# raw-lab/mercat2

Measured on AMD Instinct MI355X. Metric: bases/sec at k=31, 10Mx150bp, higher is better.
Workload: dtype u64

## Files before the change

mercat2_amd/csrc/mk_fparse.hip:

```cpp
#include "mk_common.h"
#include "mk_device.h"
#include "mk_env.h"

typedef unsigned long long u64;

#define FP_THREADS 256
#ifndef FP_SUB
#define FP_SUB 8
#endif
#define FP_WAVE_BYTES (FP_SUB * 1024)
#define FP_WAVES (FP_THREADS / 64)

struct FpEntry {
  unsigned a;
  unsigned b;
};
#define FP_A_SEPS(a) (((a) >> 2) & 0x1FFFu)
#define FP_A_FACTS 15
#define FP_F_CONV 0xFu
#define FP_F_LOW_HEAD (1u << 4)
#define FP_F_LOW_TAIL (1u << 5)
#define FP_F_HI (1u << 6)
static_assert(FP_SUB <= 15 && FP_WAVE_BYTES / 2 <= 0x1FFF, "FpEntry.a: bit fields");

__device__ __forceinline__ uint4 load16(const uint8_t* __restrict__ raw, size_t pos, size_t begin, size_t n) {
  uint4 v;
  if (pos + 16 <= n && pos >= begin) {
    v = *reinterpret_cast<const uint4*>(raw + pos);
  } else {
    unsigned w0 = 0, w1 = 0, w2 = 0, w3 = 0;
#pragma unroll
    for (int j = 0; j < 16; ++j) {
      const unsigned c = (pos + j < n && pos + j >= begin) ? (unsigned)raw[pos + j] : 10u;
      const unsigned sh = 8 * (j & 3);
      if (j < 4) w0 |= c << sh; else if (j < 8) w1 |= c << sh; else if (j < 12) w2 |= c << sh; else w3 |= c << sh;
    }
    v = make_uint4(w0, w1, w2, w3);
  }
  return v;
}

__device__ __forceinline__ void classify16(const uint4 v, unsigned& nl, unsigned& gt, unsigned& st, unsigned& low, unsigned& hi) {
#define FP_NZ7(t) ((((t) & 0x7F7F7F7Fu) + 0x7F7F7F7Fu) | (t))
  unsigned a_nl[2] = {0, 0}, a_gt[2] = {0, 0}, a_st[2] = {0, 0}, a_lo[2] = {0, 0}, a_hi[2] = {0, 0};
#pragma unroll
  for (int d = 0; d < 4; ++d) {
    const unsigned xd = d == 0 ? v.x : (d == 1 ? v.y : (d == 2 ? v.z : v.w));
    const unsigned K = (d & 1) ? 0x80402010u : 0x08040201u;
    const unsigned notnl = FP_NZ7(xd ^ 0x0A0A0A0Au) & FP_NZ7(xd ^ 0x0D0D0D0Du);
    const unsigned ge21 = ((xd & 0x7F7F7F7Fu) + 0x5F5F5F5Fu) | xd;
    a_nl[d >> 1] = __builtin_amdgcn_udot4(~notnl & 0x80808080u, K, a_nl[d >> 1], false);
    a_gt[d >> 1] = __builtin_amdgcn_udot4(~FP_NZ7(xd ^ 0x3E3E3E3Eu) & 0x80808080u, K, a_gt[d >> 1], false);
    a_st[d >> 1] = __builtin_amdgcn_udot4(~FP_NZ7(xd ^ 0x2A2A2A2Au) & 0x80808080u, K, a_st[d >> 1], false);
    a_lo[d >> 1] = __builtin_amdgcn_udot4(~ge21 & notnl & 0x80808080u, K, a_lo[d >> 1], false);
    a_hi[d >> 1] = __builtin_amdgcn_udot4(xd & 0x80808080u, K, a_hi[d >> 1], false);
  }
#undef FP_NZ7
  nl = (a_nl[0] >> 7) | ((a_nl[1] >> 7) << 8);
  gt = (a_gt[0] >> 7) | ((a_gt[1] >> 7) << 8);
  st = (a_st[0] >> 7) | ((a_st[1] >> 7) << 8);
  low = (a_lo[0] >> 7) | ((a_lo[1] >> 7) << 8);
  hi = (a_hi[0] >> 7) | ((a_hi[1] >> 7) << 8);
}

__device__ __forceinline__ unsigned lane_header(unsigned start, unsigned nl, unsigned hin, unsigned& hout) {
  const unsigned p = ~nl & 0xFFFFu;
  const unsigned a = start | p, b = start;
  const unsigned sum = a + b + hin;
  const unsigned ci = sum ^ a ^ b;
  hout = (ci >> 16) & 1u;
  return (ci >> 1) & 0xFFFFu;
}

__device__ __forceinline__ unsigned wave_step(unsigned nl, unsigned gt, unsigned st, unsigned low, unsigned prev_nl,
                                              unsigned cin, unsigned& out, unsigned& sep, unsigned& bad_low,
                                              unsigned& last_nl) {
  const int lane = threadIdx.x & 63;
  const unsigned my_last_nl = (nl >> 15) & 1u;
  const unsigned prev = (unsigned)__builtin_amdgcn_update_dpp((int)prev_nl, (int)my_last_nl, 0x138, 0xf, 0xf, false);
  const unsigned ls = ((nl << 1) | prev) & 0xFFFFu;
  const unsigned start = ls & gt;
  unsigned hout0;
  (void)lane_header(start, nl, 0u, hout0);
  const u64 G = __ballot(hout0 != 0);
  const u64 P = __ballot(nl == 0);
  const u64 A = G | P, B = G;
  const u64 sum = A + B + (u64)cin;
  const u64 CI = sum ^ A ^ B;
  const unsigned hin = (unsigned)(CI >> lane) & 1u;
  unsigned hout;
  const unsigned H = lane_header(start, nl, hin, hout);
  sep = start;
  out = ((~H & ~nl & ~st) | start) & 0xFFFFu;
  bad_low = low & ~H;
  last_nl = mk_wave_last(my_last_nl);
  return mk_wave_last(hout);
}

__global__ __launch_bounds__(FP_THREADS) void mk_fparse_summ(const uint8_t* __restrict__ raw, size_t begin, size_t n, size_t nwaves,
                                                             FpEntry* __restrict__ entries, unsigned* __restrict__ masks,
                                                             MkChunkInfo* __restrict__ info, u64* __restrict__ zero_codes,
                                                             u64* __restrict__ zero_bad, size_t code_words, size_t bad_words) {
  const size_t wave = (size_t)blockIdx.x * FP_WAVES + (threadIdx.x >> 6);
  if (wave >= nwaves) return;
  const int lane = threadIdx.x & 63;
  const size_t base = wave * FP_WAVE_BYTES;
  if (zero_codes) {
    constexpr size_t CW = FP_WAVE_BYTES / 32, BW = FP_WAVE_BYTES / 64;
    const size_t c_end = wave + 1 == nwaves ? code_words : (wave + 1) * CW, b_end = wave + 1 == nwaves ? bad_words : (wave + 1) * BW;
    for (size_t w = wave * CW + (size_t)lane; w < c_end && w < code_words; w += 64) zero_codes[w] = 0ull;
    for (size_t w = wave * BW + (size_t)lane; w < b_end && w < bad_words; w += 64) zero_bad[w] = 0ull;
  }
  unsigned prev_nl = (base <= begin) ? 1u : ((raw[base - 1] == 10 || raw[base - 1] == 13) ? 1u : 0u);
  unsigned s0 = 0, s1 = 1, c0 = 0, c1 = 0, seps = 0, any_nl = 0;
  unsigned conv = 0, low_head = 0, low_tail = 0, hi_or = 0;
  unsigned* __restrict__ wmasks = masks + wave * (FP_SUB * 64) + lane;
#pragma unroll 1
  for (int sub = 0; sub < FP_SUB; ++sub) {
    const size_t pos = base + (size_t)sub * 1024 + (size_t)lane * 16;
    unsigned nl, gt, st, low, hi;
    const uint4 v = load16(raw, pos, begin, n);
    classify16(v, nl, gt, st, low, hi);
    hi_or |= v.x | v.y | v.z | v.w;
    unsigned out, sep, bl, last_nl;
    const unsigned e0 = wave_step(nl, gt, st, low, prev_nl, s0, out, sep, bl, last_nl);
    wmasks[sub * 64] = out | (sep << 16);
    c0 += __popc(out);
    seps += __popc(sep);
    if (s1 != s0) {
      unsigned out1, sep1, bl1, ln1;
      const unsigned e1 = wave_step(nl, gt, st, low, prev_nl, s1, out1, sep1, bl1, ln1);
      c1 += __popc(out1);
      s1 = e1;
      ++conv;
      low_head |= bl;
    } else {
      c1 += __popc(out);
      s1 = e0;
      low_tail |= bl;
    }
    s0 = e0;
    any_nl |= (__ballot(nl != 0) != 0) ? 1u : 0u;
    prev_nl = last_nl;
  }
  c0 = mk_wave_sum(c0);
  c1 = mk_wave_sum(c1);
  seps = mk_wave_sum(seps);
  const unsigned facts = conv | (__ballot(low_head != 0) ? FP_F_LOW_HEAD : 0u) | (__ballot(low_tail != 0) ? FP_F_LOW_TAIL : 0u) |
                         (__ballot((hi_or & 0x80808080u) != 0) ? FP_F_HI : 0u);
  if (lane == 0) {
    entries[wave].a = any_nl | (s0 << 1) | (seps << 2) | (facts << FP_A_FACTS);
    entries[wave].b = c0 | (c1 << 16);
  }
}

struct FpScan {
  u64 off;
  unsigned st;
  unsigned facts;
};

__global__ __launch_bounds__(1024) void mk_fparse_scan(const FpEntry* __restrict__ entries, size_t nwaves,
                                                       FpScan* __restrict__ scan, MkChunkInfo* __restrict__ info,
                                                       u64* __restrict__ bad) {
  const size_t per = (nwaves + 1023) / 1024;
  const size_t lo = (size_t)threadIdx.x * per, hi = (lo + per < nwaves) ? lo + per : nwaves;
  unsigned e0 = 0, e1 = 1, has = 0;
  u64 c0 = 0, c1 = 0, nsep = 0;
  for (size_t w0 = lo; w0 < hi; w0 += 8) {
    FpEntry en[8];
#pragma unroll
    for (int i = 0; i < 8; ++i) en[i] = (w0 + i < hi) ? entries[w0 + i] : FpEntry{0u, 0u};
#pragma unroll
    for (int i = 0; i < 8; ++i) {
      if (w0 + i >= hi) break;
      const unsigned wnl = en[i].a & 1u, wx0 = (en[i].a >> 1) & 1u;
      const unsigned k0 = en[i].b & 0xFFFFu, k1 = en[i].b >> 16;
      nsep += FP_A_SEPS(en[i].a);
      c0 += e0 ? k1 : k0;
      c1 += e1 ? k1 : k0;
      e0 = wnl ? wx0 : (e0 | wx0);
      e1 = wnl ? wx0 : (e1 | wx0);
      has |= wnl;
    }
  }
  __shared__ unsigned long long w_G[16], w_P[16];
  __shared__ unsigned w_cin[16];
  __shared__ u64 w_cnt[16], w_sep[16];
  const int lane = threadIdx.x & 63, wv = threadIdx.x >> 6;
  const u64 G = __ballot(e0 != 0), P = __ballot(has == 0);
  if (lane == 0) { w_G[wv] = G; w_P[wv] = P; }
  __syncthreads();
  if (threadIdx.x == 0) {
    unsigned cin = 0;
    for (int w = 0; w < 16; ++w) {
      w_cin[w] = cin;
      const u64 A = w_G[w] | w_P[w], B = w_G[w];
      const u64 sum = A + B + cin;
      const u64 CI = sum ^ A ^ B;
      cin = (unsigned)((w_G[w] >> 63) | ((w_P[w] >> 63) & (CI >> 63))) & 1u;
    }
  }
  __syncthreads();
  unsigned q;
  {
    const u64 A = G | P, B = G;
    const u64 CI = (A + B + (u64)w_cin[wv]) ^ A ^ B;
    q = (unsigned)(CI >> lane) & 1u;
  }
  const u64 mine = q ? c1 : c0;
  u64 inc = mine;
#pragma unroll
  for (int d = 1; d < 64; d <<= 1) {
    const u64 up = __shfl_up(inc, d);
    if (lane >= d) inc += up;
  }
  for (int d = 32; d > 0; d >>= 1) nsep += __shfl_down(nsep, d);
  if (lane == 63) w_cnt[wv] = inc;
  if (lane == 0) w_sep[wv] = nsep;
  __syncthreads();
  u64 off = inc - mine;
  u64 total = 0, seps = 0;
#pragma unroll
  for (int w = 0; w < 16; ++w) {
    const u64 v = w_cnt[w];
    if (w < wv) off += v;
    total += v;
    seps += w_sep[w];
  }
  if (threadIdx.x == 0) {
    info->seq_len = total;
    info->symbols = total - seps;
    if (bad) {
      if (total & 63) atomicOr(&bad[total >> 6], ~0ull << (total & 63));
      const u64 w = (total + 63) >> 6;
      bad[w] = ~0ull;
      bad[w + 1] = ~0ull;
      bad[w + 2] = ~0ull;
    }
  }
  for (size_t w0 = lo; w0 < hi; w0 += 8) {
    FpEntry en[8];
#pragma unroll
    for (int i = 0; i < 8; ++i) en[i] = (w0 + i < hi) ? entries[w0 + i] : FpEntry{0u, 0u};
#pragma unroll
    for (int i = 0; i < 8; ++i) {
      if (w0 + i >= hi) break;
      scan[w0 + i].off = off;
      scan[w0 + i].st = q;
      scan[w0 + i].facts = en[i].a >> FP_A_FACTS;
      const unsigned wnl = en[i].a & 1u, wx0 = (en[i].a >> 1) & 1u;
      off += q ? (en[i].b >> 16) : (en[i].b & 0xFFFFu);
      q = wnl ? wx0 : (q | wx0);
    }
  }
}

__global__ __launch_bounds__(FP_THREADS) void mk_fparse_emit(const uint8_t* __restrict__ raw, size_t begin, size_t n, size_t nwaves,
                                                             const FpScan* __restrict__ scan, const unsigned* __restrict__ masks,
                                                             uint8_t* __restrict__ seq, MkChunkInfo* __restrict__ info,
                                                             u64* __restrict__ codes, u64* __restrict__ bad, int write_seq,
                                                             int classic) {
  __shared__ __attribute__((aligned(16))) uint8_t stage[FP_WAVES][64 + FP_WAVE_BYTES + 32 + 64 + 256];
  const int wv = threadIdx.x >> 6;
  const size_t wave = (size_t)blockIdx.x * FP_WAVES + wv;
  if (wave >= nwaves) return;
  const int lane = threadIdx.x & 63;
  const size_t base = wave * FP_WAVE_BYTES;
  const FpScan sc = scan[wave];
  const unsigned shift = (unsigned)(sc.off & 15);
  uint8_t* __restrict__ lds = stage[wv] + 64;
  const bool all_classic = classic || (sc.facts & FP_F_HI);
  const int nclassic = __builtin_amdgcn_readfirstlane(all_classic ? FP_SUB : (sc.st ? (int)(sc.facts & FP_F_CONV) : 0));
  unsigned prev_nl = (nclassic == 0 || base <= begin) ? 1u : ((raw[base - 1] == 10 || raw[base - 1] == 13) ? 1u : 0u);
  unsigned state = sc.st;
  unsigned filled = 0;
  int nbad = 0;
  unsigned flag_low = all_classic ? 0u : (sc.facts & (sc.st ? FP_F_LOW_TAIL : (FP_F_LOW_TAIL | FP_F_LOW_HEAD)));
  unsigned nhi = 0;
  const unsigned* __restrict__ wmasks = masks + wave * (FP_SUB * 64) + lane;
  uint4 v_next = load16(raw, base + (size_t)lane * 16, begin, n);
  unsigned m_next = wmasks[0];
#pragma unroll 1
  for (int sub = 0; sub < FP_SUB; ++sub) {
    const uint4 v = v_next;
    const unsigned m = m_next;
    if (sub + 1 < FP_SUB) {
      v_next = load16(raw, base + (size_t)(sub + 1) * 1024 + (size_t)lane * 16, begin, n);
      m_next = wmasks[(sub + 1) * 64];
    }
    unsigned out, sep;
    if (sub < nclassic) {
      unsigned nl, gt, st, low, hi, bl, last_nl;
      classify16(v, nl, gt, st, low, hi);
      state = wave_step(nl, gt, st, low, prev_nl, state, out, sep, bl, last_nl);
      prev_nl = last_nl;
      flag_low |= bl;
      nhi += __popc(hi & out & ~sep);
    } else {
      out = m & 0xFFFFu;
      sep = m >> 16;
    }
    const unsigned cnt = __popc(out);
    nbad -= (int)__popc(sep);
    const unsigned inc = mk_wave_scan_incl(cnt);
    unsigned at = shift + filled + inc - cnt;
#define FP_BYTE(j) ((uint8_t)(((j) < 4 ? v.x : ((j) < 8 ? v.y : ((j) < 12 ? v.z : v.w))) >> (8 * ((j) & 3))))
    if (out == 0xFFFFu && sep == 0) {
#ifdef FP_BYTE_STORES
#pragma unroll
      for (int j = 0; j < 16; ++j) lds[at + j] = FP_BYTE(j);
#else
      __builtin_memcpy(lds + at, &v, 16);
#endif
    } else if (out) {
      const unsigned dump = FP_WAVE_BYTES + 32 + 64 + ((unsigned)lane << 2);
      unsigned a = at;
#pragma unroll
      for (int j = 0; j < 16; ++j) {
        const unsigned kept = (out >> j) & 1u;
        lds[kept ? a : dump] = FP_BYTE(j);
        a += kept;
      }
      for (unsigned sp = sep; sp; sp &= sp - 1) lds[at + __popc(out & ((1u << (__ffs(sp) - 1)) - 1u))] = (uint8_t)MK_SEP;
    }
#undef FP_BYTE
    filled += mk_wave_last(inc);
  }
  __builtin_amdgcn_wave_barrier();
  __threadfence_block();
  uint8_t* __restrict__ dst = seq + (sc.off - shift);
  const unsigned end = shift + filled;
  for (unsigned c = (unsigned)lane * 16; write_seq && c < end; c += 64 * 16) {
    if (c >= shift && c + 16 <= end) {
      *reinterpret_cast<uint4*>(dst + c) = *reinterpret_cast<const uint4*>(lds + c);
    } else {
      const unsigned lo = c < shift ? shift : c;
      const unsigned hi = c + 16 < end ? c + 16 : end;
      for (unsigned j = lo; j < hi; ++j) dst[j] = lds[j];
    }
  }
  if (codes) {
    const u64 g0 = sc.off, g1 = sc.off + filled;
    for (u64 b = (g0 >> 6) + lane; b < ((g1 + 63) >> 6); b += 64) {
      const u64 s_lo = b << 6, s_hi = s_lo + 64;
      const u64 lo = s_lo > g0 ? s_lo : g0, hi = s_hi < g1 ? s_hi : g1;
      u64 w0 = 0, w1 = 0, bd = 0;
      unsigned b8[8] = {0, 0, 0, 0, 0, 0, 0, 0};
      const uint4* p = reinterpret_cast<const uint4*>(lds + (long)shift + (long)(s_lo - g0));
#pragma unroll
      for (int q = 0; q < 4; ++q) {
        const uint4 v = p[q];
#pragma unroll
        for (int d = 0; d < 4; ++d) {
          const unsigned xd = d == 0 ? v.x : (d == 1 ? v.y : (d == 2 ? v.z : v.w));
          const unsigned c = ((xd >> 1) & 0x03030303u) ^ ((xd >> 2) & 0x01010101u);
          const unsigned df = __builtin_amdgcn_perm(0u, 0x54474341u, c) ^ xd;
          const unsigned nz = (((df & 0x7F7F7F7Fu) + 0x7F7F7F7Fu) | df) & 0x80808080u;
          const unsigned m1 = nz >> 7;
          const unsigned ck = c & ~(m1 | (m1 << 1));
          const unsigned g = __builtin_amdgcn_udot4(ck, 0x01041040u, 0u, false);
          const int idx = q * 4 + d;
          if (idx < 8) w0 |= (u64)g << (56 - 8 * idx); else w1 |= (u64)g << (56 - 8 * (idx - 8));
          b8[idx >> 1] = __builtin_amdgcn_udot4(nz, (idx & 1) ? 0x80402010u : 0x08040201u, b8[idx >> 1], false);
        }
      }
#pragma unroll
      for (int i = 0; i < 8; ++i) bd |= (u64)(b8[i] >> 7) << (8 * i);
      if (hi - lo == 64) {
        codes[2 * b] = w0;
        codes[2 * b + 1] = w1;
        bad[b] = bd;
      } else {
        const unsigned a = (unsigned)(lo - s_lo), e = (unsigned)(hi - s_lo);
        const u64 inmask = ((e - a) >= 64 ? ~0ull : ((1ull << (e - a)) - 1)) << a;
        const unsigned a0 = a < 32 ? a : 32, e0 = e < 32 ? e : 32, a1 = a > 32 ? a - 32 : 0, e1 = e > 32 ? e - 32 : 0;
        const u64 m0 = a0 < e0 ? ((~0ull >> (2 * a0)) & ~(e0 == 32 ? 0ull : (~0ull >> (2 * e0)))) : 0ull;
        const u64 m1 = a1 < e1 ? ((~0ull >> (2 * a1)) & ~(e1 == 32 ? 0ull : (~0ull >> (2 * e1)))) : 0ull;
        w0 &= m0;
        w1 &= m1;
        bd &= inmask;
        if (w0) atomicOr(&codes[2 * b], w0);
        if (w1) atomicOr(&codes[2 * b + 1], w1);
        if (bd) atomicOr(&bad[b], bd);
      }
      nbad += (int)__popcll(bd);
    }
  }
  for (int d = 32; d > 0; d >>= 1) nbad += __shfl_down(nbad, d);
  if (codes && lane == 0 && nbad > 0) atomicAdd(&info->bad_symbols, (u64)nbad);
  if (__ballot(flag_low != 0) && lane == 0) atomicOr(&info->parse_fallback, 1ull);
  if (__ballot(nhi != 0)) {
    for (int d = 32; d > 0; d >>= 1) nhi += __shfl_down(nhi, d);
    if (lane == 0) atomicAdd(&info->non_ascii, (u64)nhi);
  }
}

int mk_launch_fparse(mk_ctx* c, const uint8_t* d_raw, size_t begin, size_t len, bool fuse_pack_nt, bool write_seq) {
  if (!fuse_pack_nt) write_seq = true;
  const size_t n = begin + len;
  u64* codes = fuse_pack_nt ? (u64*)c->codes.p : nullptr;
  u64* bad = fuse_pack_nt ? (u64*)c->bad.p : nullptr;
  const size_t bad_words = n / 64 + 4;
  if (fuse_pack_nt && len == 0) {
    MK_HIP(hipMemsetAsync(c->codes.p, 0, 2 * bad_words * sizeof(u64), c->stream));
    MK_HIP(hipMemsetAsync(c->bad.p, 0, bad_words * sizeof(u64), c->stream));
    if (n == 0) MK_HIP(hipMemsetAsync(c->bad.p, 0xFF, 4 * sizeof(u64), c->stream));
  }
  if (len == 0) return MK_OK;
  const size_t nwaves = (n + FP_WAVE_BYTES - 1) / FP_WAVE_BYTES;
  const size_t e_bytes = (nwaves * sizeof(FpEntry) + 15) & ~(size_t)15;
  const size_t m_off = (e_bytes + nwaves * sizeof(FpScan) + 255) & ~(size_t)255;
  int rc = mk_buf_reserve(c, c->tile_maps, m_off + nwaves * FP_SUB * 64 * sizeof(unsigned));
  if (rc) return rc;
  FpEntry* entries = (FpEntry*)c->tile_maps.p;
  FpScan* scan = (FpScan*)((char*)c->tile_maps.p + e_bytes);
  unsigned* masks = (unsigned*)((char*)c->tile_maps.p + m_off);
  MkChunkInfo* info = (MkChunkInfo*)c->info.p;
  const unsigned blocks = (unsigned)((nwaves + FP_WAVES - 1) / FP_WAVES);
  const bool classic = mk_env_int("MK_FP_CLASSIC", 0) != 0;
  mk_prof_begin(c, MK_K_PARSE);
  hipLaunchKernelGGL(mk_fparse_summ, dim3(blocks), dim3(FP_THREADS), 0, c->stream, d_raw, begin, n, nwaves, entries, masks, info, codes,
                     bad, 2 * bad_words, bad_words);
  hipLaunchKernelGGL(mk_fparse_scan, dim3(1), dim3(1024), 0, c->stream, (const FpEntry*)entries, nwaves, scan, info, bad);
  hipLaunchKernelGGL(mk_fparse_emit, dim3(blocks), dim3(FP_THREADS), 0, c->stream, d_raw, begin, n, nwaves, (const FpScan*)scan,
                     (const unsigned*)masks, (uint8_t*)c->seq.p, info, codes, bad, write_seq ? 1 : 0, classic ? 1 : 0);
  mk_prof_end(c);
  MK_HIP(hipGetLastError());
  return MK_OK;
}
```

Before: 173.6 billion.

## Pack 2-bit codes and bad masks directly in emit, skipping LDS byte compaction

Adds a templated symbolic emit path used when codes are requested and the sequence bytes are not written. Each lane encodes its 16 bytes into 2-bit codes and bad bits and ORs them into per-wave LDS code and bad images at the compacted offsets using LDS atomics. The images are then written to global memory, with atomics only on boundary words. This removes the byte staging pass and the second pass that re-reads LDS to pack codes, at the cost of LDS atomics per run of kept bytes and a zero-clear of the images.

```diff
diff --git a/mercat2_amd/csrc/mk_fparse.hip b/mercat2_amd/csrc/mk_fparse.hip
--- a/mercat2_amd/csrc/mk_fparse.hip
+++ b/mercat2_amd/csrc/mk_fparse.hip
@@ -256,20 +256,33 @@
   }
 }
 
+#define FP_SYM_CODE_U32 (FP_WAVE_BYTES / 16 + 8)
+#define FP_SYM_BAD_U32 (FP_WAVE_BYTES / 32 + 4)
+static_assert(FP_SYM_CODE_U32 % 4 == 0 && FP_SYM_BAD_U32 % 4 == 0, "the staging image is cleared 16 bytes a lane");
+template <bool SYM>
 __global__ __launch_bounds__(FP_THREADS) void mk_fparse_emit(const uint8_t* __restrict__ raw, size_t begin, size_t n, size_t nwaves,
                                                              const FpScan* __restrict__ scan, const unsigned* __restrict__ masks,
                                                              uint8_t* __restrict__ seq, MkChunkInfo* __restrict__ info,
                                                              u64* __restrict__ codes, u64* __restrict__ bad, int write_seq,
                                                              int classic) {
-  __shared__ __attribute__((aligned(16))) uint8_t stage[FP_WAVES][64 + FP_WAVE_BYTES + 32 + 64 + 256];
+  constexpr unsigned STAGE_BYTES = SYM ? (FP_SYM_CODE_U32 + FP_SYM_BAD_U32) * 4 : 64 + FP_WAVE_BYTES + 32 + 64 + 256;
+  __shared__ __attribute__((aligned(16))) uint8_t stage[FP_WAVES][STAGE_BYTES];
   const int wv = threadIdx.x >> 6;
   const size_t wave = (size_t)blockIdx.x * FP_WAVES + wv;
   if (wave >= nwaves) return;
   const int lane = threadIdx.x & 63;
   const size_t base = wave * FP_WAVE_BYTES;
   const FpScan sc = scan[wave];
-  const unsigned shift = (unsigned)(sc.off & 15);
-  uint8_t* __restrict__ lds = stage[wv] + 64;
+  const unsigned shift = (unsigned)(sc.off & (SYM ? 63 : 15));
+  uint8_t* __restrict__ lds = stage[wv] + (SYM ? 0 : 64);
+  unsigned* __restrict__ cimg = reinterpret_cast<unsigned*>(stage[wv]);
+  unsigned* __restrict__ bimg = cimg + FP_SYM_CODE_U32;
+  if (SYM) {
+    for (unsigned i = (unsigned)lane; i < (FP_SYM_CODE_U32 + FP_SYM_BAD_U32) / 4; i += 64)
+      reinterpret_cast<uint4*>(stage[wv])[i] = make_uint4(0u, 0u, 0u, 0u);
+    __builtin_amdgcn_wave_barrier();
+    __threadfence_block();
+  }
   const bool all_classic = classic || (sc.facts & FP_F_HI);
   const int nclassic = __builtin_amdgcn_readfirstlane(all_classic ? FP_SUB : (sc.st ? (int)(sc.facts & FP_F_CONV) : 0));
   unsigned prev_nl = (nclassic == 0 || base <= begin) ? 1u : ((raw[base - 1] == 10 || raw[base - 1] == 13) ? 1u : 0u);
@@ -305,6 +318,40 @@
     nbad -= (int)__popc(sep);
     const unsigned inc = mk_wave_scan_incl(cnt);
     unsigned at = shift + filled + inc - cnt;
+    if constexpr (SYM) {
+      unsigned code32 = 0, f8[2] = {0, 0};
+#pragma unroll
+      for (int d = 0; d < 4; ++d) {
+        const unsigned xd = d == 0 ? v.x : (d == 1 ? v.y : (d == 2 ? v.z : v.w));
+        const unsigned c = ((xd >> 1) & 0x03030303u) ^ ((xd >> 2) & 0x01010101u);
+        const unsigned df = __builtin_amdgcn_perm(0u, 0x54474341u, c) ^ xd;
+        const unsigned nz = (((df & 0x7F7F7F7Fu) + 0x7F7F7F7Fu) | df) & 0x80808080u;
+        const unsigned m1 = nz >> 7;
+        const unsigned ck = c & ~(m1 | (m1 << 1));
+        code32 |= __builtin_amdgcn_udot4(ck, 0x01041040u, 0u, false) << (24 - 8 * d);
+        f8[d >> 1] = __builtin_amdgcn_udot4(nz, (d & 1) ? 0x80402010u : 0x08040201u, f8[d >> 1], false);
+      }
+      const unsigned bad16 = (f8[0] >> 7) | ((f8[1] >> 7) << 8);
+      for (unsigned m = out; m; ) {
+        const unsigned s = (unsigned)__ffs(m) - 1u;
+        const unsigned r = (unsigned)__ffs(~(m >> s)) - 1u;
+        const unsigned cv = ((code32 << (2 * s)) >> (32 - 2 * r)) << (32 - 2 * r);
+        const u64 cx = ((u64)cv << 32) >> (2 * (at & 15));
+        const unsigned L = at >> 4;
+        if ((unsigned)(cx >> 32)) atomicOr(&cimg[L ^ 1u], (unsigned)(cx >> 32));
+        if ((unsigned)cx) atomicOr(&cimg[(L + 1u) ^ 1u], (unsigned)cx);
+        const unsigned bv = (bad16 >> s) & ((1u << r) - 1u);
+        if (bv) {
+          const u64 bx = (u64)bv << (at & 31);
+          atomicOr(&bimg[at >> 5], (unsigned)bx);
+          if ((unsigned)(bx >> 32)) atomicOr(&bimg[(at >> 5) + 1u], (unsigned)(bx >> 32));
+        }
+        at += r;
+        m &= m + (1u << s);
+      }
+      filled += mk_wave_last(inc);
+      continue;
+    }
 #define FP_BYTE(j) ((uint8_t)(((j) < 4 ? v.x : ((j) < 8 ? v.y : ((j) < 12 ? v.z : v.w))) >> (8 * ((j) & 3))))
     if (out == 0xFFFFu && sep == 0) {
 #ifdef FP_BYTE_STORES
@@ -329,9 +376,28 @@
   }
   __builtin_amdgcn_wave_barrier();
   __threadfence_block();
+  if constexpr (SYM) {
+    const u64 g0 = sc.off, g1 = sc.off + filled;
+    const u64 b0 = g0 >> 6;
+    for (u64 b = b0 + lane; b < ((g1 + 63) >> 6); b += 64) {
+      const unsigned i = (unsigned)(b - b0);
+      const uint4 cw = reinterpret_cast<const uint4*>(cimg)[i];
+      const u64 bd = reinterpret_cast<const u64*>(bimg)[i];
+      if ((b << 6) >= g0 && (b << 6) + 64 <= g1) {
+        *reinterpret_cast<uint4*>(codes + 2 * b) = cw;
+        bad[b] = bd;
+      } else {
+        const u64 w0 = ((u64)cw.y << 32) | cw.x, w1 = ((u64)cw.w << 32) | cw.z;
+        if (w0) atomicOr(&codes[2 * b], w0);
+        if (w1) atomicOr(&codes[2 * b + 1], w1);
+        if (bd) atomicOr(&bad[b], bd);
+      }
+      nbad += (int)__popcll(bd);
+    }
+  }
   uint8_t* __restrict__ dst = seq + (sc.off - shift);
   const unsigned end = shift + filled;
-  for (unsigned c = (unsigned)lane * 16; write_seq && c < end; c += 64 * 16) {
+  for (unsigned c = (unsigned)lane * 16; !SYM && write_seq && c < end; c += 64 * 16) {
     if (c >= shift && c + 16 <= end) {
       *reinterpret_cast<uint4*>(dst + c) = *reinterpret_cast<const uint4*>(lds + c);
     } else {
@@ -340,7 +406,7 @@
       for (unsigned j = lo; j < hi; ++j) dst[j] = lds[j];
     }
   }
-  if (codes) {
+  if (!SYM && codes) {
     const u64 g0 = sc.off, g1 = sc.off + filled;
     for (u64 b = (g0 >> 6) + lane; b < ((g1 + 63) >> 6); b += 64) {
       const u64 s_lo = b << 6, s_hi = s_lo + 64;
@@ -419,12 +485,17 @@
   MkChunkInfo* info = (MkChunkInfo*)c->info.p;
   const unsigned blocks = (unsigned)((nwaves + FP_WAVES - 1) / FP_WAVES);
   const bool classic = mk_env_int("MK_FP_CLASSIC", 0) != 0;
+  const bool sym = codes != nullptr && !write_seq && mk_env_int("MK_FP_BYTES", 0) == 0;
   mk_prof_begin(c, MK_K_PARSE);
   hipLaunchKernelGGL(mk_fparse_summ, dim3(blocks), dim3(FP_THREADS), 0, c->stream, d_raw, begin, n, nwaves, entries, masks, info, codes,
                      bad, 2 * bad_words, bad_words);
   hipLaunchKernelGGL(mk_fparse_scan, dim3(1), dim3(1024), 0, c->stream, (const FpEntry*)entries, nwaves, scan, info, bad);
-  hipLaunchKernelGGL(mk_fparse_emit, dim3(blocks), dim3(FP_THREADS), 0, c->stream, d_raw, begin, n, nwaves, (const FpScan*)scan,
-                     (const unsigned*)masks, (uint8_t*)c->seq.p, info, codes, bad, write_seq ? 1 : 0, classic ? 1 : 0);
+  if (sym)
+    hipLaunchKernelGGL(mk_fparse_emit<true>, dim3(blocks), dim3(FP_THREADS), 0, c->stream, d_raw, begin, n, nwaves, (const FpScan*)scan,
+                       (const unsigned*)masks, (uint8_t*)c->seq.p, info, codes, bad, 0, classic ? 1 : 0);
+  else
+    hipLaunchKernelGGL(mk_fparse_emit<false>, dim3(blocks), dim3(FP_THREADS), 0, c->stream, d_raw, begin, n, nwaves, (const FpScan*)scan,
+                       (const unsigned*)masks, (uint8_t*)c->seq.p, info, codes, bad, write_seq ? 1 : 0, classic ? 1 : 0);
   mk_prof_end(c);
   MK_HIP(hipGetLastError());
   return MK_OK;
```

Measured after the change: 171.8 billion. 0.99x the previous value.
